# arkworks-rs/circom-compat

Hardware: NVIDIA H100
Metric: groth16_proofs_per_sec_bn254_2p20 (higher is better)
Workload: dtype u32x8 (254-bit Montgomery integers)

## Files before the change

### circom_compat_b200/csrc/msm.cu

```cuda
#include <type_traits>
#include "msm.cuh"
#include "util.cuh"

namespace b2g {

std::atomic<uint64_t> g_launch_count{0};

template <class C, class F>
__global__ void __launch_bounds__(128) msm_table_kernel(const void* __restrict__ bases, uint32_t n, int c, int nwin, void* __restrict__ table) {
    uint32_t i = blockIdx.x * blockDim.x + threadIdx.x;
    if (i >= n) return;
    using Pt = typename C::Pt; using Aff = typename C::Aff; using E = typename F::elem;
    Aff p = aff_load<F>(bases, i);
    if (C::aff_is_inf(p)) {
        Aff z; z.x = F::zero(); z.y = F::zero();
        for (int w = 0; w < nwin; w++) aff_store<F>(table, (size_t)w * n + i, z);
        return;
    }
    Pt pts[MSM_MAX_WIN];
    E pre[MSM_MAX_WIN];
    Pt cur = C::from_affine(p);
    E acc = F::one();
    for (int w = 0; w < nwin; w++) {
        pts[w] = cur;
// ... 81 lines not shown
        if (mine) pending = false;
    }
    if (pending) atomicAdd(&counts[b], 1u);
}

__global__ void __launch_bounds__(1024) msm_scan_kernel(const uint32_t* __restrict__ counts, uint32_t nb, uint32_t* __restrict__ offsets,
                                                        uint32_t* __restrict__ cursor) {
    __shared__ uint32_t warp_sums[32];
    __shared__ uint32_t carry_s;
    const uint32_t tid = threadIdx.x, per = (nb + 1023u) / 1024u;
    const uint32_t lo = tid * per, hi = min(lo + per, nb);
    uint32_t s = 0;
    if ((per & 3u) == 0 && hi == lo + per) {
        const uint4* v4 = reinterpret_cast<const uint4*>(counts + lo);
        #pragma unroll 4
        for (uint32_t j = 0; j < per / 4; j++) { const uint4 q = __ldg(&v4[j]); s += q.x + q.y + q.z + q.w; }
    } else {
        for (uint32_t j = lo; j < hi; j++) s += counts[j];
    }
    uint32_t v = s;
    #pragma unroll
    for (int d = 1; d < 32; d <<= 1) { uint32_t t = __shfl_up_sync(0xffffffffu, v, d); if ((tid & 31) >= (uint32_t)d) v += t; }
    if ((tid & 31) == 31) warp_sums[tid >> 5] = v;
    __syncthreads();
    if (tid < 32) {
        uint32_t w = warp_sums[tid], x = w;
        #pragma unroll
        for (int d = 1; d < 32; d <<= 1) { uint32_t t = __shfl_up_sync(0xffffffffu, x, d); if (tid >= (uint32_t)d) x += t; }
        warp_sums[tid] = x - w;
        if (tid == 31) carry_s = x;
    }
    __syncthreads();
    uint32_t run = warp_sums[tid >> 5] + v - s;
    for (uint32_t j = lo; j < hi; j++) { offsets[j] = run; cursor[j] = 0; run += counts[j]; }
    if (tid == 0) offsets[nb] = carry_s;
}

__global__ void __launch_bounds__(256) msm_scatter_kernel(const fe* __restrict__ canon, uint32_t n, uint32_t row_stride, int c, int nwin, uint32_t nb,
                                   const uint32_t* __restrict__ offsets, uint32_t* __restrict__ cursor, uint32_t* __restrict__ entries) {
    canon += (size_t)blockIdx.y * n;
    offsets += (size_t)blockIdx.y * nb;
    cursor += (size_t)blockIdx.y * nb;
    const uint64_t tid = (uint64_t)blockIdx.x * blockDim.x + threadIdx.x;
    const uint32_t w = (uint32_t)(tid / n), i = (uint32_t)(tid % n);
    int32_t d = 0;
    if (w < (uint32_t)nwin) d = msm_digit_at(canon[i].l, c, (int)w);
    const uint32_t b = d ? (uint32_t)(d < 0 ? -d : d) - 1u : 0xffffffffu;
    const uint32_t lane = threadIdx.x & 31;
    const uint32_t entry = (w * row_stride + i) | (d < 0 ? 0x80000000u : 0u);
    bool pending = d != 0;
    {
        const uint32_t hot = __ballot_sync(0xffffffffu, pending && b == 0u);
        if (hot) {
            const int leader = __ffs(hot) - 1;
            uint32_t base = 0;
            if ((int)lane == leader) base = atomicAdd(&cursor[0], (uint32_t)__popc(hot));
            base = __shfl_sync(0xffffffffu, base, leader);
            if (pending && b == 0u) {
                entries[offsets[0] + base + (uint32_t)__popc(hot & ((1u << lane) - 1u))] = entry;
                pending = false;
            }
        }
    }
    #pragma unroll
    for (int round = 0; round < MSM_LEADER_ROUNDS; round++) {
        const uint32_t pend = __ballot_sync(0xffffffffu, pending);
        if (!pend) break;
        const int leader = __ffs(pend) - 1;
        const uint32_t lb = __shfl_sync(0xffffffffu, b, leader);
        const bool mine = pending && b == lb;
        const uint32_t same = __ballot_sync(0xffffffffu, mine);
        uint32_t base = 0;
        if ((int)lane == leader) base = atomicAdd(&cursor[lb], (uint32_t)__popc(same));
        base = __shfl_sync(0xffffffffu, base, leader);
        if (mine) {
            entries[offsets[b] + base + (uint32_t)__popc(same & ((1u << lane) - 1u))] = entry;
            pending = false;
        }
    }
    if (pending) entries[offsets[b] + atomicAdd(&cursor[b], 1u)] = entry;
}


__device__ __forceinline__ void acc_stage_slab(uint32_t* slab, unsigned long long* slab_bar, const uint32_t* __restrict__ entries,
                                               uint64_t cta_first, uint32_t total, uint32_t slab_words) {
    const uint32_t bar = (uint32_t)__cvta_generic_to_shared(slab_bar);
    if (threadIdx.x == 0) {
        asm volatile("mbarrier.init.shared::cta.b64 [%0], 1;" :: "r"(bar));
        asm volatile("fence.mbarrier_init.release.cluster;" ::: "memory");
    }
    __syncthreads();
    if (threadIdx.x == 0 && cta_first < total) {
        const uint64_t left = total - cta_first;
        const uint32_t bytes = (uint32_t)(((left < slab_words ? left : (uint64_t)slab_words) * 4 + 15) & ~15ull);
        asm volatile("mbarrier.arrive.expect_tx.shared::cta.b64 _, [%0], %1;" :: "r"(bar), "r"(bytes) : "memory");
        asm volatile("cp.async.bulk.shared::cluster.global.mbarrier::complete_tx::bytes [%0], [%1], %2, [%3];"
                     :: "r"((uint32_t)__cvta_generic_to_shared(slab)), "l"(entries + cta_first), "r"(bytes), "r"(bar) : "memory");
    }
    if (cta_first < total) {
        uint32_t done = 0;
        while (!done)
            asm volatile("{\n\t.reg .pred p;\n\tmbarrier.try_wait.parity.shared::cta.b64 p, [%1], 0;\n\tselp.u32 %0, 1, 0, p;\n\t}" : "=r"(done) : "r"(bar) : "memory");
    }
}

constexpr int MSM_SLAB_MAX_BYTES = 48 * 1024;

__device__ __forceinline__ uint32_t acc_first_bucket(const uint32_t* __restrict__ offsets, uint32_t nb, uint32_t start, uint32_t& bucket_end) {
    uint32_t lo = 0, hi = nb;
    while (hi - lo > 1) { uint32_t mid = (lo + hi) >> 1; if (offsets[mid] <= start) lo = mid; else hi = mid; }
    uint32_t b = lo;
    bucket_end = offsets[b + 1];
    while (bucket_end <= start) { b++; bucket_end = offsets[b + 1]; }
    return b;
}

template <class C, class F>
__global__ void __launch_bounds__(128, 4) msm_accumulate_kernel(const void* __restrict__ table, const uint32_t* __restrict__ entries,
                                      const uint32_t* __restrict__ offsets, uint32_t nb, uint32_t chunk,
                                      void* __restrict__ buckets, void* __restrict__ frag_first, void* __restrict__ frag_last, uint32_t slab_words) {
    using Pt = typename C::Pt; using Aff = typename C::Aff;
    const uint32_t total = offsets[nb];
    const uint32_t t = blockIdx.x * blockDim.x + threadIdx.x;
    const uint64_t start64 = (uint64_t)t * chunk;
    extern __shared__ __align__(128) uint32_t slab[];
    __shared__ __align__(8) unsigned long long slab_bar;
    const uint64_t cta_first = (uint64_t)blockIdx.x * blockDim.x * chunk;
    if (slab_words) acc_stage_slab(slab, &slab_bar, entries, cta_first, total, slab_words);
    if (start64 >= total) return;
    const uint32_t start = (uint32_t)start64;
    const uint32_t end = (uint32_t)min((uint64_t)total, start64 + chunk);
    uint32_t bucket_end;
    uint32_t b = acc_first_bucket(offsets, nb, start, bucket_end);
    Pt acc = C::infinity();
    uint32_t seg_start = start;
    for (uint32_t pos = start; pos < end;) {
        const uint32_t e = slab_words ? slab[pos - start + threadIdx.x * chunk] : entries[pos];
        Aff p = aff_load<F>(table, (size_t)(e & 0x7fffffffu));
        if (e >> 31) p.y = F::neg(p.y);
        C::madd(acc, p);
        pos++;
        if (pos == bucket_end || pos == end) {
            const uint32_t bucket_start = offsets[b];
            if (bucket_start >= start && bucket_end <= end) pt_store<F>(buckets, b, acc);
            else if (seg_start == start) pt_store<F>(frag_first, t, acc);
            else pt_store<F>(frag_last, t, acc);
            acc = C::infinity();
            seg_start = pos;
            if (pos == bucket_end && pos < end) {
                do { b++; bucket_end = offsets[b + 1]; } while (bucket_end <= pos);
            }
        }
    }
}

__global__ void __launch_bounds__(128, 3) msm_accumulate_g2_kernel(const void* __restrict__ table, const uint32_t* __restrict__ entries,
                                      const uint32_t* __restrict__ offsets, uint32_t nb, uint32_t chunk,
                                      void* __restrict__ buckets, void* __restrict__ frag_first, void* __restrict__ frag_last) {
    const uint32_t total = offsets[nb];
    const uint32_t t = (blockIdx.x * blockDim.x + threadIdx.x) >> 1;
    const uint32_t half = threadIdx.x & 1u;
    const bool A = half == 0;
    const unsigned mask = 3u << (threadIdx.x & 30u);
    const uint64_t start64 = (uint64_t)t * chunk;
    if (start64 >= total) return;
    const uint32_t start = (uint32_t)start64;
    const uint32_t end = (uint32_t)min((uint64_t)total, start64 + chunk);
    uint32_t bucket_end;
    uint32_t b = acc_first_bucket(offsets, nb, start, bucket_end);
    fe2 s0 = Fq2::zero(), s1 = Fq2::zero();
    bool empty = true;
    uint32_t seg_start = start;
    for (uint32_t pos = start; pos < end;) {
        const uint32_t e = entries[pos];
        fe2 qc;
        elem_load_nc(qc, (const char*)table + (size_t)(e & 0x7fffffffu) * 128 + half * 64);
        qc = Fq2::sel((e >> 31) && !A, Fq2::neg(qc), qc);
        G2Pair::madd(s0, s1, empty, qc, A, mask);
        pos++;
        if (pos == bucket_end || pos == end) {
            const uint32_t bucket_start = offsets[b];
            char* rec;
            if (bucket_start >= start && bucket_end <= end) rec = (char*)buckets + (size_t)b * 256;
            else if (seg_start == start) rec = (char*)frag_first + (size_t)t * 256;
            else rec = (char*)frag_last + (size_t)t * 256;
            elem_store(rec + half * 64, s0);
            elem_store(rec + 128 + half * 64, s1);
            s0 = Fq2::zero(); s1 = Fq2::zero(); empty = true;
            seg_start = pos;
            if (pos == bucket_end && pos < end) {
                do { b++; bucket_end = offsets[b + 1]; } while (bucket_end <= pos);
            }
        }
    }
}


template <class C, class F>
__global__ void __launch_bounds__(128) msm_fold_kernel(const uint32_t* __restrict__ offsets, uint32_t nb, uint32_t chunk, void* __restrict__ buckets,
                                const void* __restrict__ frag_first, const void* __restrict__ frag_last,
                                uint32_t* __restrict__ big_list, uint32_t* __restrict__ big_count) {
    using Pt = typename C::Pt;
    uint32_t b = blockIdx.x * blockDim.x + threadIdx.x;
    if (b >= nb) return;
    uint32_t s = offsets[b], e = offsets[b + 1];
    if (s == e) { pt_store<F>(buckets, b, C::infinity()); return; }
    uint32_t t0 = s / chunk, t1 = (e - 1) / chunk;
    if (t0 == t1) return;
    if (t1 - t0 + 1 > (uint32_t)MSM_BIG_FRAGS) { big_list[atomicAdd(big_count, 1u)] = b; return; }
    Pt acc = (s == t0 * chunk) ? pt_load<F>(frag_first, t0) : pt_load<F>(frag_last, t0);
    for (uint32_t t = t0 + 1; t <= t1; t++) { Pt q = pt_load<F>(frag_first, t); C::add(acc, q); }
    pt_store<F>(buckets, b, acc);
}

template <class F> struct PtWords;
template <> struct PtWords<Fq> { static constexpr int N = 32; };
template <> struct PtWords<Fq2> { static constexpr int N = 64; };

template <class C, class F>
__device__ __forceinline__ typename C::Pt warp_sum_points(typename C::Pt v) {
    using Pt = typename C::Pt;
    static_assert(sizeof(Pt) == PtWords<F>::N * 4, "XYZZ point layout");
    #pragma unroll 1
    for (int d = 16; d > 0; d >>= 1) {
        Pt q;
        uint32_t* qw = reinterpret_cast<uint32_t*>(&q);
        const uint32_t* vw = reinterpret_cast<const uint32_t*>(&v);
        #pragma unroll
        for (int i = 0; i < PtWords<F>::N; i++) qw[i] = __shfl_down_sync(0xffffffffu, vw[i], d);
        if ((int)(threadIdx.x & 31) < d) C::add(v, q);
    }
    return v;
}

template <class C, class F, int NT>
__device__ __forceinline__ typename C::Pt block_sum_points(typename C::Pt v, typename C::Pt* sh) {
    static_assert(NT == 32 || NT == 64, "one or two warps");
    v = warp_sum_points<C, F>(v);
    if (NT == 32) return v;
    if ((threadIdx.x & 31) == 0) sh[threadIdx.x >> 5] = v;
    __syncthreads();
    if (threadIdx.x == 0) { typename C::Pt q = sh[1]; C::add(v, q); }
    __syncthreads();
    return v;
}

template <class F> struct TailThreads;
template <> struct TailThreads<Fq> { static constexpr int N = 64; };
template <> struct TailThreads<Fq2> { static constexpr int N = 32; };
constexpr int MSM_REDUCE_CHUNK_DEFAULT = 8;

template <class C, class F>
__global__ void __launch_bounds__(TailThreads<F>::N) msm_fold_big_kernel(const uint32_t* __restrict__ offsets, uint32_t chunk, void* __restrict__ buckets,
                                    const void* __restrict__ frag_first, const void* __restrict__ frag_last,
                                    const uint32_t* __restrict__ big_list, const uint32_t* __restrict__ big_count) {
    using Pt = typename C::Pt;
    extern __shared__ __align__(32) unsigned char smem_raw[];
    Pt* sh = reinterpret_cast<Pt*>(smem_raw);
    const uint32_t nbig = *big_count;
    for (uint32_t bi = blockIdx.x; bi < nbig; bi += gridDim.x) {
        uint32_t b = big_list[bi];
// ... 28 lines not shown
            C::add(acc, run);
        }
        if (base != 0 && !C::is_inf(run)) {
            Pt m = C::infinity();
            int top = 31 - __clz(base);
            for (int i = top; i >= 0; i--) { m = C::dbl(m); if ((base >> i) & 1u) C::add(m, run); }
            C::add(acc, m);
        }
    }
    Pt r = block_sum_points<C, F, TailThreads<F>::N>(acc, sh);
    if (threadIdx.x == 0) pt_store<F>(partials, blockIdx.x, r);
}

template <class C, class F>
__global__ void __launch_bounds__(TailThreads<F>::N) msm_sum_kernel(const void* __restrict__ pts, uint32_t count, void* __restrict__ out, size_t out_stride) {
    using Pt = typename C::Pt;
    extern __shared__ __align__(32) unsigned char smem_raw[];
    Pt* sh = reinterpret_cast<Pt*>(smem_raw);
    pts = (const char*)pts + (size_t)blockIdx.x * count * sizeof(Pt);
    out = (char*)out + (size_t)blockIdx.x * out_stride;
    Pt acc = C::infinity();
    for (uint32_t i = threadIdx.x; i < count; i += TailThreads<F>::N) { Pt q = pt_load<F>(pts, i); C::add(acc, q); }
    Pt r = block_sum_points<C, F, TailThreads<F>::N>(acc, sh);
    if (threadIdx.x == 0) pt_store<F>(out, 0, r);
}

static uint32_t env_u32(const char* name, uint32_t dflt) {
    const char* v = getenv(name);
    if (!v || !*v) return dflt;
    long x = strtol(v, nullptr, 10);
    return x > 0 ? (uint32_t)x : dflt;
}

void msm_validate_points(const void* pts_dev, uint32_t n, bool g2, cudaStream_t st, const char* what) {
    if (n == 0) return;
    struct Flag { uint32_t* d = nullptr; ~Flag() { if (d) cudaFree(d); } } flag;
    uint32_t bad = 0;
    CUDA_CHECK(cudaMalloc(&flag.d, 4));
    CUDA_CHECK(cudaMemsetAsync(flag.d, 0, 4, st));
    if (g2) msm_validate_kernel<G2, Fq2><<<(n + 255) / 256, 256, 0, st>>>(pts_dev, n, flag.d);
    else msm_validate_kernel<G1, Fq><<<(n + 255) / 256, 256, 0, st>>>(pts_dev, n, flag.d);
    g_launch_count += 1;
    CUDA_CHECK(cudaMemcpyAsync(&bad, flag.d, 4, cudaMemcpyDeviceToHost, st));
    CUDA_CHECK(cudaStreamSynchronize(st));
    if (bad) throw_error(B2G_E_INPUT, std::string(g2 ? "G2" : "G1") + " point " + std::to_string(bad - 1) + " of " + what + " is not on the curve");
}

template <class C, class F>
static void msm_build_table_t(MsmPlan& plan, const void* bases_dev, uint32_t n, cudaStream_t st) {
    const size_t aff = 2 * Bytes<F>::ELEM;
    uint32_t c = env_u32("B2G_MSM_C", (uint32_t)msm_pick_c(n ? n : 1));
    if (c < 8 || c > 22) throw_error(B2G_E_SHAPE, "B2G_MSM_C must be in [8, 22]");
    plan.n = n; plan.c = (int)c; plan.nwin = msm_nwin(plan.c); plan.nbuckets = 1u << (plan.c - 1);
    if (n == 0) { plan.table = nullptr; return; }
    if ((uint64_t)n * plan.nwin >= (1ull << 31)) throw_error(B2G_E_SHAPE, "msm: n * windows exceeds 2^31 table rows");
    msm_validate_points(bases_dev, n, plan.g2, st, "the query slice");
    CUDA_CHECK(cudaMalloc(&plan.table, (size_t)n * plan.nwin * aff));
    msm_table_kernel<C, F><<<(n + 127) / 128, 128, 0, st>>>(bases_dev, n, plan.c, plan.nwin, plan.table);
    g_launch_count += 1;
    CUDA_CHECK(cudaGetLastError());
}

void msm_build_table(MsmPlan& plan, const void* bases_dev, uint32_t n, bool g2, cudaStream_t st) {
    plan.g2 = g2;
    if (g2) msm_build_table_t<G2, Fq2>(plan, bases_dev, n, st);
    else msm_build_table_t<G1, Fq>(plan, bases_dev, n, st);
}

void msm_free_table(MsmPlan& plan) { if (plan.table) cudaFree(plan.table); plan.table = nullptr; }

void msm_scratch_alloc(MsmScratch& s, uint32_t n, int nwin, uint32_t nbuckets_one, bool g2, bool with_sort, uint32_t count) {
    s.g2 = g2; s.cap_n = n; s.cap_nwin = nwin; s.cap_buckets = nbuckets_one; s.cap_count = count;
    s.chunk = env_u32(g2 ? "B2G_MSM_CHUNK_G2" : "B2G_MSM_CHUNK", env_u32("B2G_MSM_CHUNK", 64));
    const size_t pt = (g2 ? 4 * 64 : 4 * 32);
    const size_t nent = (size_t)n * nwin * count;
    const size_t nbuckets = (size_t)nbuckets_one * count;
    const size_t nchunks = (nent + s.chunk - 1) / s.chunk + 1;
    s.reduce_chunk = env_u32("B2G_MSM_REDUCE_CHUNK", MSM_REDUCE_CHUNK_DEFAULT);
    const size_t npart = ((size_t)nbuckets_one / (s.reduce_chunk * 32) + 64) * count;
    if (with_sort) {
        CUDA_CHECK(cudaMalloc(&s.counts, (size_t)nbuckets * 4));
        CUDA_CHECK(cudaMalloc(&s.offsets, ((size_t)nbuckets + 1) * 4));
        CUDA_CHECK(cudaMalloc(&s.cursor, (size_t)nbuckets * 4));
        CUDA_CHECK(cudaMalloc(&s.entries, (nent + 8) * 4));
        CUDA_CHECK(cudaMalloc(&s.scalars_canon, ((size_t)n * count + 1) * sizeof(fe)));
    }
    CUDA_CHECK(cudaMalloc(&s.big_list, (size_t)nbuckets * 4));
    CUDA_CHECK(cudaMalloc(&s.big_count, 4));
    CUDA_CHECK(cudaMalloc(&s.frag_first, nchunks * pt));
    CUDA_CHECK(cudaMalloc(&s.frag_last, nchunks * pt));
    CUDA_CHECK(cudaMalloc(&s.buckets, (size_t)nbuckets * pt));
    CUDA_CHECK(cudaMalloc(&s.partials, (npart + 1) * pt));
    CUDA_CHECK(cudaMalloc(&s.result, pt)); s.result_owned = true;
    int least = 0, greatest = 0;
    CUDA_CHECK(cudaDeviceGetStreamPriorityRange(&least, &greatest));
    CUDA_CHECK(cudaStreamCreateWithPriority(&s.tail, cudaStreamNonBlocking, greatest));
    CUDA_CHECK(cudaEventCreateWithFlags(&s.ev_acc, cudaEventDisableTiming));
    CUDA_CHECK(cudaEventCreateWithFlags(&s.ev_tail, cudaEventDisableTiming));
}

void msm_scratch_free(MsmScratch& s) {
    void* ptrs[] = {s.counts, s.offsets, s.cursor, s.entries, s.big_list, s.big_count, s.frag_first, s.frag_last,
                    s.buckets, s.partials, s.result_owned ? s.result : nullptr, s.scalars_canon};
    for (void* p : ptrs) if (p) cudaFree(p);
    if (s.tail) { cudaStreamDestroy(s.tail); cudaEventDestroy(s.ev_acc); cudaEventDestroy(s.ev_tail); }
    s = MsmScratch();
}

void msm_sort(const MsmPlan& plan, MsmScratch& s, const fe* scalars_dev, uint32_t n, bool scalars_mont, cudaStream_t st, uint32_t count,
              uint32_t scalar_stride) {
    if (n > plan.n) n = plan.n;
    s.sorted_n = n; s.sorted_count = count;
    if (n == 0 || plan.table == nullptr) return;
    if (n > s.cap_n || plan.nwin > s.cap_nwin || plan.nbuckets > s.cap_buckets || count > s.cap_count || !s.entries) throw_error(B2G_E_SHAPE, "msm: sort scratch too small");
    const uint32_t nb = plan.nbuckets * count;
    constexpr unsigned SORT_CTA = 256;
    CUDA_CHECK(cudaMemsetAsync(s.counts, 0, (size_t)nb * 4, st));
    const dim3 pair_grid((unsigned)(((uint64_t)n * plan.nwin + SORT_CTA - 1) / SORT_CTA), count);
    msm_canon_kernel<<<dim3((n + SORT_CTA - 1) / SORT_CTA, count), SORT_CTA, 0, st>>>(scalars_dev, n, scalar_stride ? scalar_stride : n, scalars_mont ? 1 : 0, s.scalars_canon);
    msm_count_kernel<<<pair_grid, SORT_CTA, 0, st>>>(s.scalars_canon, n, plan.c, plan.nwin, plan.nbuckets, s.counts);
    msm_scan_kernel<<<1, 1024, 0, st>>>(s.counts, nb, s.offsets, s.cursor);
    msm_scatter_kernel<<<pair_grid, SORT_CTA, 0, st>>>(s.scalars_canon, n, plan.n, plan.c, plan.nwin, plan.nbuckets, s.offsets, s.cursor, s.entries);
    g_launch_count += 4;
    CUDA_CHECK(cudaGetLastError());
}

template <class C, class F>
static void launch_accumulate(const void* table, const uint32_t* entries, const uint32_t* offsets, uint32_t nb, uint32_t chunk, uint32_t nruns,
                              const MsmScratch& s, cudaStream_t st) {
    constexpr bool g2 = std::is_same<F, Fq2>::value;
    constexpr uint32_t runs_per_cta = g2 ? 64u : 128u;
    const unsigned blocks = (unsigned)(((uint64_t)nruns + runs_per_cta - 1) / runs_per_cta);
    if constexpr (g2) {
        msm_accumulate_g2_kernel<<<blocks, 128, 0, st>>>(table, entries, offsets, nb, chunk, s.buckets, s.frag_first, s.frag_last);
    } else {
        const uint32_t slab_words = (size_t)chunk * runs_per_cta * 4 <= MSM_SLAB_MAX_BYTES ? chunk * runs_per_cta : 0u;
        msm_accumulate_kernel<C, F><<<blocks, 128, (size_t)slab_words * 4, st>>>(table, entries, offsets, nb, chunk, s.buckets, s.frag_first, s.frag_last, slab_words);
    }
}

template <class C, class F>
static void msm_accumulate_t(const MsmPlan& plan, const MsmScratch& sorted, MsmScratch& s, cudaStream_t st) {
    using Pt = typename C::Pt;
    const size_t ptb = sizeof(Pt);
    const uint32_t n = sorted.sorted_n, count = sorted.sorted_count;
    const size_t rstride = s.result_stride ? s.result_stride : ptb;
    if (n == 0 || plan.table == nullptr) { CUDA_CHECK(cudaMemset2DAsync(s.result, rstride, 0, ptb, count, st)); return; }
    if (plan.nbuckets > s.cap_buckets || n > s.cap_n || plan.nwin > s.cap_nwin || count > s.cap_count) throw_error(B2G_E_SHAPE, "msm: accumulate scratch too small");
    const uint32_t nb = plan.nbuckets * count, chunk = s.chunk;
    const uint32_t* offsets = sorted.offsets;
    CUDA_CHECK(cudaMemsetAsync(s.big_count, 0, 4, st));
    const uint64_t nent = (uint64_t)n * plan.nwin * count;
    const uint32_t nthreads = (uint32_t)((nent + chunk - 1) / chunk);
    if (s.prof0) CUDA_CHECK(cudaEventRecord(s.prof0, st));
    launch_accumulate<C, F>(plan.table, sorted.entries, offsets, nb, chunk, nthreads, s, st);
    if (s.prof1) CUDA_CHECK(cudaEventRecord(s.prof1, st));
    cudaStream_t main_st = st;
    CUDA_CHECK(cudaEventRecord(s.ev_acc, st)); CUDA_CHECK(cudaStreamWaitEvent(s.tail, s.ev_acc, 0)); st = s.tail;
    msm_fold_kernel<C, F><<<(nb + 127) / 128, 128, 0, st>>>(offsets, nb, chunk, s.buckets, s.frag_first, s.frag_last, s.big_list, s.big_count);
    constexpr int NT = TailThreads<F>::N;
    const size_t sh = (size_t)NT * ptb;
    msm_fold_big_kernel<C, F><<<128, NT, sh, st>>>(offsets, chunk, s.buckets, s.frag_first, s.frag_last, s.big_list, s.big_count);
    const uint32_t rchunk = s.reduce_chunk, nb1 = plan.nbuckets;
    const uint32_t nred = (nb1 + rchunk - 1) / rchunk;
    const uint32_t npart = (nred + NT - 1) / NT;
    msm_reduce_kernel<C, F><<<dim3(npart, count), NT, sh, st>>>(s.buckets, nb1, rchunk, s.partials);
    msm_sum_kernel<C, F><<<count, NT, sh, st>>>(s.partials, npart, s.result, rstride);
    CUDA_CHECK(cudaEventRecord(s.ev_tail, s.tail)); CUDA_CHECK(cudaStreamWaitEvent(main_st, s.ev_tail, 0));
    g_launch_count += 5;
    CUDA_CHECK(cudaGetLastError());
}

void msm_accumulate(const MsmPlan& plan, const MsmScratch& sorted, MsmScratch& acc, cudaStream_t st) {
    if (plan.g2) msm_accumulate_t<G2, Fq2>(plan, sorted, acc, st);
    else msm_accumulate_t<G1, Fq>(plan, sorted, acc, st);
}

void msm_run(const MsmPlan& plan, MsmScratch& s, const fe* scalars_dev, uint32_t n, bool scalars_mont, cudaStream_t st, uint32_t count,
             uint32_t scalar_stride) {
    msm_sort(plan, s, scalars_dev, n, scalars_mont, st, count, scalar_stride);
    msm_accumulate(plan, s, s, st);
}

constexpr uint32_t POWERS_CHUNK = 16;

__global__ void powers_base_kernel(const fe* __restrict__ rho, uint64_t start, fe* __restrict__ pw) {
    if (threadIdx.x != 0 || blockIdx.x != 0) return;
    const fe r = *rho;
    fe acc = Fr::one(), sq = r;
    for (uint64_t e = start; e; e >>= 1) {
        if (e & 1) acc = Fr::mul(acc, sq);
        sq = Fr::sqr(sq);
    }
    pw[0] = acc;
    fe c = r;
    for (uint32_t k = 1; k < POWERS_CHUNK; k <<= 1) c = Fr::sqr(c);
    pw[1] = c;
}

__global__ void __launch_bounds__(256) powers_scalars_kernel(const fe* __restrict__ rho, const fe* __restrict__ pw, uint32_t n,
                                                             fe* __restrict__ canon) {
    const uint32_t t = blockIdx.x * blockDim.x + threadIdx.x;
    const uint32_t i0 = t * POWERS_CHUNK;
    if (i0 >= n) return;
    fe x = pw[0], sq = pw[1];
    for (uint32_t e = t; e; e >>= 1) {
        if (e & 1) x = Fr::mul(x, sq);
        sq = Fr::sqr(sq);
    }
    const fe r = *rho;
    const uint32_t end = min(n, i0 + POWERS_CHUNK);
    for (uint32_t i = i0; i < end; i++) {
        fe_store(&canon[i], Fr::to_canonical(x));
        x = Fr::mul(x, r);
    }
}

__global__ void __launch_bounds__(256) powers_count_kernel(const fe* __restrict__ canon, uint32_t n, int c, int nwin, uint32_t nb,
                                                           uint32_t* __restrict__ counts) {
    const uint64_t tid = (uint64_t)blockIdx.x * blockDim.x + threadIdx.x;
    const uint32_t w = (uint32_t)(tid / n), i = (uint32_t)(tid % n);
    if (w >= (uint32_t)nwin) return;
    const int32_t d = msm_digit_at(canon[i].l, c, (int)w);
    if (d) atomicAdd(&counts[w * nb + (uint32_t)(d < 0 ? -d : d) - 1u], 1u);
}

__global__ void __launch_bounds__(256) powers_scatter_kernel(const fe* __restrict__ canon, uint32_t n, int c, int nwin, uint32_t nb,
                                                             const uint32_t* __restrict__ offsets, uint32_t* __restrict__ cursor,
                                                             uint32_t* __restrict__ entries) {
    const uint64_t tid = (uint64_t)blockIdx.x * blockDim.x + threadIdx.x;
    const uint32_t w = (uint32_t)(tid / n), i = (uint32_t)(tid % n);
    if (w >= (uint32_t)nwin) return;
    const int32_t d = msm_digit_at(canon[i].l, c, (int)w);
    if (!d) return;
    const uint32_t key = w * nb + (uint32_t)(d < 0 ? -d : d) - 1u;
    entries[offsets[key] + atomicAdd(&cursor[key], 1u)] = i | (d < 0 ? 0x80000000u : 0u);
}

template <class C, class F>
__global__ void powers_horner_kernel(const void* __restrict__ windows, int nwin, int c, void* __restrict__ acc) {
    if (threadIdx.x != 0 || blockIdx.x != 0) return;
    typename C::Pt r = pt_load<F>(windows, nwin - 1);
    for (int w = nwin - 2; w >= 0; w--) {
        for (int k = 0; k < c; k++) r = C::dbl(r);
        C::add(r, pt_load<F>(windows, w));
    }
    typename C::Pt a = pt_load<F>(acc, 0);
    C::add(a, r);
    pt_store<F>(acc, 0, a);
}

void powers_msm_alloc(PowersMsm& m, bool g2, uint32_t cap) {
    m.g2 = g2;
    m.cap = cap ? cap : 1;
    m.c = powers_pick_c(m.cap);
    m.nwin = msm_nwin(m.c);
    m.nbuckets = 1u << (m.c - 1);
    const size_t pt = g2 ? 256 : 128, nb = (size_t)m.nbuckets * m.nwin;
    msm_scratch_alloc(m.s, m.cap, 1, m.nbuckets, g2, false, (uint32_t)m.nwin);
    CUDA_CHECK(cudaMalloc(&m.s.counts, nb * 4));
    CUDA_CHECK(cudaMalloc(&m.s.offsets, (nb + 1) * 4));
    CUDA_CHECK(cudaMalloc(&m.s.cursor, nb * 4));
    CUDA_CHECK(cudaMalloc(&m.s.entries, ((size_t)m.cap * m.nwin + 8) * 4));
    CUDA_CHECK(cudaMalloc(&m.s.scalars_canon, ((size_t)m.cap + POWERS_CHUNK) * sizeof(fe)));
    CUDA_CHECK(cudaFree(m.s.result));
    m.s.result = nullptr;
    CUDA_CHECK(cudaMalloc(&m.s.result, (size_t)m.nwin * pt));
    m.s.result_stride = pt;
    CUDA_CHECK(cudaMalloc(&m.acc, pt));
    CUDA_CHECK(cudaMalloc(&m.pw, 2 * sizeof(fe)));
}

void powers_msm_free(PowersMsm& m) {
    msm_scratch_free(m.s);
    if (m.acc) cudaFree(m.acc);
    if (m.pw) cudaFree(m.pw);
    m = PowersMsm();
}

void powers_msm_reset(PowersMsm& m, cudaStream_t st) { CUDA_CHECK(cudaMemsetAsync(m.acc, 0, m.g2 ? 256 : 128, st)); }

void powers_scalars(const fe* rho, uint64_t start, uint32_t n, fe* pw, fe* canon, cudaStream_t st) {
    if (n == 0) return;
    constexpr unsigned CTA = 256;
    powers_base_kernel<<<1, 1, 0, st>>>(rho, start, pw);
    powers_scalars_kernel<<<(n + POWERS_CHUNK * CTA - 1) / (POWERS_CHUNK * CTA), CTA, 0, st>>>(rho, pw, n, canon);
    g_launch_count += 2;
    CUDA_CHECK(cudaGetLastError());
}

template <class C, class F>
static void powers_msm_slice_t(PowersMsm& m, const void* bases, uint32_t n, uint64_t start, const fe* rho, cudaStream_t st,
                               const fe* scalars) {
    if (n == 0) return;
    if (n > m.cap) throw_error(B2G_E_SHAPE, "powers msm: slice larger than its buffers");
    constexpr unsigned CTA = 256;
    const uint32_t nb = m.nbuckets * (uint32_t)m.nwin;
    if (!scalars) {
        powers_scalars(rho, start, n, m.pw, m.s.scalars_canon, st);
        scalars = m.s.scalars_canon;
    }
    CUDA_CHECK(cudaMemsetAsync(m.s.counts, 0, (size_t)nb * 4, st));
    const unsigned blocks = (unsigned)(((uint64_t)n * m.nwin + CTA - 1) / CTA);
    powers_count_kernel<<<blocks, CTA, 0, st>>>(scalars, n, m.c, m.nwin, m.nbuckets, m.s.counts);
    msm_scan_kernel<<<1, 1024, 0, st>>>(m.s.counts, nb, m.s.offsets, m.s.cursor);
    powers_scatter_kernel<<<blocks, CTA, 0, st>>>(scalars, n, m.c, m.nwin, m.nbuckets, m.s.offsets, m.s.cursor, m.s.entries);
    g_launch_count += 3;
    CUDA_CHECK(cudaGetLastError());
    MsmPlan plan;
    plan.n = n; plan.c = m.c; plan.nwin = 1; plan.nbuckets = m.nbuckets; plan.table = const_cast<void*>(bases); plan.g2 = m.g2;
    m.s.sorted_n = n; m.s.sorted_count = (uint32_t)m.nwin;
    msm_accumulate_t<C, F>(plan, m.s, m.s, st);
    powers_horner_kernel<C, F><<<1, 1, 0, st>>>(m.s.result, m.nwin, m.c, m.acc);
    g_launch_count += 1;
    CUDA_CHECK(cudaGetLastError());
}

void powers_msm_slice(PowersMsm& m, const void* bases, uint32_t n, uint64_t start, const fe* rho, cudaStream_t st, const fe* scalars) {
    if (m.g2) powers_msm_slice_t<G2, Fq2>(m, bases, n, start, rho, st, scalars);
    else powers_msm_slice_t<G1, Fq>(m, bases, n, start, rho, st, scalars);
}

void msm_init_kernels() {
    CUDA_CHECK(cudaFuncSetAttribute(msm_accumulate_kernel<G1, Fq>, cudaFuncAttributeMaxDynamicSharedMemorySize, MSM_SLAB_MAX_BYTES));
}

}
```

### circom_compat_b200/csrc/prover.cu

```cuda
#include <atomic>
#include <chrono>
#include <cstring>
#include <vector>
#include "../../include/b2groth.h"
#include "ec.cuh"
#include "msm.cuh"
#include "fixed.cuh"
#include "ntt.cuh"
#include "setup.cuh"
#include "util.cuh"
#include "verify.cuh"

namespace b2g {

void msm_build_table(MsmPlan& plan, const void* bases_dev, uint32_t n, bool g2, cudaStream_t st);
void msm_free_table(MsmPlan& plan);
void msm_scratch_alloc(MsmScratch& s, uint32_t n, int nwin, uint32_t nbuckets, bool g2, bool with_sort, uint32_t count = 1);
void msm_sort(const MsmPlan& plan, MsmScratch& s, const fe* scalars_dev, uint32_t n, bool scalars_mont, cudaStream_t st, uint32_t count = 1,
              uint32_t scalar_stride = 0);
void msm_accumulate(const MsmPlan& plan, const MsmScratch& sorted, MsmScratch& acc, cudaStream_t st);
void msm_scratch_free(MsmScratch& s);
void msm_run(const MsmPlan& plan, MsmScratch& s, const fe* scalars_dev, uint32_t n, bool scalars_mont, cudaStream_t st, uint32_t count = 1,
             uint32_t scalar_stride = 0);
void msm_init_kernels();
void msm_validate_points(const void* pts_dev, uint32_t n, bool g2, cudaStream_t st, const char* what);

enum { Q_H = 0, Q_L = 1, Q_A = 2, Q_B1 = 3, Q_B2 = 4, NQ = 5 };
static const size_t PARTIAL_OFF[NQ] = {0, 128, 256, 384, 512};
constexpr size_t REC_BYTES = B2G_PARTIAL_BYTES + 256;
constexpr uint32_t MAX_BATCH = 65535;

}

using namespace b2g;

struct b2g_ctx {
    int device = 0, shard_rank = 0, shard_count = 1;
    cudaStream_t st[NQ] = {}, st_glue = nullptr;
    cudaEvent_t ev_w = nullptr, ev_sort = nullptr, ev_pre = nullptr, ev_fork = nullptr, ev_done[NQ] = {}, ev_t[20] = {};
    MsmScratch scratch[NQ];
    bool scratch_ok = false;
    uint32_t cap_batch = 1;
    uint8_t* d_partial = nullptr;
    uint8_t* d_partials_all = nullptr;
    uint8_t* d_proof = nullptr;
    uint8_t* d_pre = nullptr;
    fe *d_w = nullptr, *d_a = nullptr, *d_b = nullptr, *d_c = nullptr, *d_h = nullptr;
    fe* d_wb = nullptr; size_t cap_wb = 0;
    cudaEvent_t ev_sortb = nullptr; bool scratch_bsort = false;
    size_t cap_w = 0, cap_n = 0;
    float last_ms[16] = {};
    bool pre_valid = false; uint32_t pre_r[8] = {}, pre_s[8] = {};
    uint8_t *d_rs = nullptr, *h_rs = nullptr;
    uint8_t *h_proof = nullptr, *pending_out = nullptr;
    uint32_t pending_count = 0;
    bool use_graph = true;
    cudaGraphExec_t gexec[2] = {nullptr, nullptr};
    uint64_t g_key[2][4] = {};
    uint64_t alloc_gen = 1;
    uint64_t g_launches[2] = {0, 0};
    unsigned long long* d_epoch = nullptr;
    uint8_t* d_xchg = nullptr;
    size_t eval_cap = 0, eval_common = 0;
    uint8_t** d_peer_ptrs = nullptr;
    void* peer_mapped[64] = {};
    int peers_imported = 0;
    VerifyBufs* vbufs = nullptr;
};

static std::atomic<uint64_t> g_next_uid{1};

struct b2g_pk {
    uint64_t uid = g_next_uid++;
    int device = 0, shard_rank = 0, shard_count = 1;
    uint32_t n_vars = 0, n_public = 0, domain = 0;
    MsmPlan plan[NQ];
    uint32_t lo[NQ] = {}, cnt[NQ] = {}, scalar_off[NQ] = {};
    uint8_t* d_consts = nullptr;
    void *d_tab_delta1 = nullptr, *d_tab_delta2 = nullptr;
    void *d_tab_aa = nullptr, *d_tab_bb = nullptr;
    uint32_t* d_bidx = nullptr;
    uint32_t b_compact = 0;
};

struct b2g_mat {
    uint64_t uid = g_next_uid++;
    int device = 0;
    uint32_t m = 0, num_inputs = 0, n_vars = 0, n = 0;
    int logn = 0;
    NttDomain dom;
    uint32_t *a_rowptr = nullptr, *a_col = nullptr, *b_rowptr = nullptr, *b_col = nullptr, *c_rowptr = nullptr, *c_col = nullptr;
    fe *a_val = nullptr, *b_val = nullptr, *c_val = nullptr;
    uint32_t reduction = B2G_REDUCTION_CIRCOM;
};

namespace b2g {

thread_local std::string g_last_error;

struct Scalar256 { uint32_t l[8]; };

CtxView ctx_view(b2g_ctx* ctx) { return {ctx->device, ctx->st[0], ctx->pending_out != nullptr, &ctx->vbufs}; }

constexpr size_t PRE_BYTES = 2 * 128 + 256;
__global__ void __launch_bounds__(160) glue_pre_kernel(const void* __restrict__ tab_d1, const void* __restrict__ tab_d2, const void* __restrict__ tab_aa,
                                                       const void* __restrict__ tab_bb, const Scalar256* __restrict__ rs, uint8_t* __restrict__ pre) {
    __shared__ G1::Pt sh1[4][32];
// ... 534 lines not shown
    if (!ctx->use_graph) { enqueue_proof(ctx, pk, mat, kind, true, count); return; }
    const uint64_t key[4] = {pk->uid, mat->uid, ctx->alloc_gen, count};
    if (ctx->gexec[kind] && memcmp(ctx->g_key[kind], key, sizeof key)) { cudaGraphExecDestroy(ctx->gexec[kind]); ctx->gexec[kind] = nullptr; }
    if (!ctx->gexec[kind]) {
        const uint64_t before = g_launch_count.load();
        cudaGraph_t graph = nullptr;
        CUDA_CHECK(cudaStreamBeginCapture(s0, cudaStreamCaptureModeThreadLocal));
        try { enqueue_proof(ctx, pk, mat, kind, false, count); }
        catch (...) { cudaStreamEndCapture(s0, &graph); if (graph) cudaGraphDestroy(graph); cudaGetLastError(); g_launch_count = before; throw; }
        cudaError_t e = cudaStreamEndCapture(s0, &graph);
        if (e == cudaSuccess) e = cudaGraphInstantiate(&ctx->gexec[kind], graph, 0);
        if (graph) cudaGraphDestroy(graph);
        ctx->g_launches[kind] = g_launch_count.load() - before;
        g_launch_count = before;
        if (e != cudaSuccess) {
            cudaGetLastError();
            ctx->gexec[kind] = nullptr; ctx->use_graph = false;
            enqueue_proof(ctx, pk, mat, kind, true, count);
            return;
        }
        memcpy(ctx->g_key[kind], key, sizeof key);
    }
    CUDA_CHECK(cudaEventRecord(ctx->ev_t[10], s0)); CUDA_CHECK(cudaEventRecord(ctx->ev_t[11], s0));
    for (int i = 0; i < 10; i++) CUDA_CHECK(cudaEventRecord(ctx->ev_t[i], s0));
    CUDA_CHECK(cudaGraphLaunch(ctx->gexec[kind], s0));
    CUDA_CHECK(cudaEventRecord(ctx->ev_t[14], s0));
    g_launch_count += ctx->g_launches[kind];
}

static void collect_timings(b2g_ctx* ctx) {
    auto el = [&](int a, int b) { float ms = 0; cudaEventElapsedTime(&ms, ctx->ev_t[a], ctx->ev_t[b]); return ms; };
    ctx->last_ms[0] = el(12, 13);
    ctx->last_ms[1] = el(10, 11);
    ctx->last_ms[2] = el(0, 1);
    for (int q = 1; q < NQ; q++) ctx->last_ms[2 + q] = el(2 * q, 2 * q + 1);
    ctx->last_ms[7] = el(14, 15);
    ctx->last_ms[8] = el(12, 15);
}

}

extern "C" {

const char* b2g_last_error(void) { return g_last_error.c_str(); }
int b2g_version(void) { return 1; }

int b2g_device_count(int* count) {
    return guarded([&] { if (!count) throw_error(B2G_E_SHAPE, "null pointer"); CUDA_CHECK(cudaGetDeviceCount(count)); });
}

int b2g_ctx_create(int device, int shard_rank, int shard_count, b2g_ctx** out) {
    return guarded([&] {
        if (!out) throw_error(B2G_E_SHAPE, "null pointer");
        if (shard_count < 1 || shard_count > 64 || shard_rank < 0 || shard_rank >= shard_count) throw_error(B2G_E_SHAPE, "bad shard rank/count");
        int ndev = 0;
        CUDA_CHECK(cudaGetDeviceCount(&ndev));
        if (device < 0 || device >= ndev) throw_error(B2G_E_DEVICE, "no such CUDA device (this library has no CPU fallback)");
        DevGuard g(device);
        b2g_ctx* ctx = new b2g_ctx();
        ctx->device = device; ctx->shard_rank = shard_rank; ctx->shard_count = shard_count;
        int least = 0, greatest = 0;
        CUDA_CHECK(cudaDeviceGetStreamPriorityRange(&least, &greatest));
        for (int i = 0; i < NQ; i++) { CUDA_CHECK(cudaStreamCreateWithPriority(&ctx->st[i], cudaStreamNonBlocking, least)); CUDA_CHECK(cudaEventCreateWithFlags(&ctx->ev_done[i], cudaEventDisableTiming)); }
        CUDA_CHECK(cudaEventCreateWithFlags(&ctx->ev_w, cudaEventDisableTiming));
        CUDA_CHECK(cudaEventCreateWithFlags(&ctx->ev_sort, cudaEventDisableTiming));
        CUDA_CHECK(cudaEventCreateWithFlags(&ctx->ev_pre, cudaEventDisableTiming));
        CUDA_CHECK(cudaEventCreateWithFlags(&ctx->ev_fork, cudaEventDisableTiming));
        CUDA_CHECK(cudaEventCreateWithFlags(&ctx->ev_sortb, cudaEventDisableTiming));
        CUDA_CHECK(cudaStreamCreateWithPriority(&ctx->st_glue, cudaStreamNonBlocking, least));
        for (auto& e : ctx->ev_t) CUDA_CHECK(cudaEventCreate(&e));
        CUDA_CHECK(cudaMalloc(&ctx->d_partial, REC_BYTES));
        CUDA_CHECK(cudaMemset(ctx->d_partial, 0, REC_BYTES));
        CUDA_CHECK(cudaMalloc(&ctx->d_partials_all, 64 * REC_BYTES));
        CUDA_CHECK(cudaMalloc(&ctx->d_proof, 256));
        CUDA_CHECK(cudaMalloc(&ctx->d_pre, PRE_BYTES));
        CUDA_CHECK(cudaMalloc(&ctx->d_rs, 64));
        CUDA_CHECK(cudaMallocHost(&ctx->h_rs, 64));
        CUDA_CHECK(cudaMallocHost(&ctx->h_proof, 256));
        CUDA_CHECK(cudaMalloc(&ctx->d_epoch, 8));
        CUDA_CHECK(cudaMemset(ctx->d_epoch, 0, 8));
        { const char* g = getenv("B2G_GRAPH"); ctx->use_graph = !(g && *g == '0'); }
        cudaDeviceSetLimit(cudaLimitMaxL2FetchGranularity, 64); cudaGetLastError();
        CUDA_CHECK(cudaMalloc(&ctx->d_peer_ptrs, 64 * sizeof(uint8_t*)));
        msm_init_kernels();
        *out = ctx;
    });
}

int b2g_ctx_destroy(b2g_ctx* ctx) {
    return guarded([&] {
        if (!ctx) return;
        DevGuard g(ctx->device);
        cudaDeviceSynchronize();
        for (int i = 0; i < NQ; i++) { if (ctx->scratch_ok) msm_scratch_free(ctx->scratch[i]); cudaStreamDestroy(ctx->st[i]); cudaEventDestroy(ctx->ev_done[i]); }
        cudaEventDestroy(ctx->ev_w); cudaEventDestroy(ctx->ev_sort); cudaEventDestroy(ctx->ev_pre); cudaEventDestroy(ctx->ev_fork); cudaEventDestroy(ctx->ev_sortb); cudaStreamDestroy(ctx->st_glue);
        if (ctx->d_wb) cudaFree(ctx->d_wb);
        for (auto& g : ctx->gexec) if (g) cudaGraphExecDestroy(g);
        if (ctx->h_rs) cudaFreeHost(ctx->h_rs);
        if (ctx->h_proof) cudaFreeHost(ctx->h_proof);
        if (ctx->d_rs) cudaFree(ctx->d_rs);
        if (ctx->d_epoch) cudaFree(ctx->d_epoch);
        for (auto& e : ctx->ev_t) cudaEventDestroy(e);
        for (int k = 0; k < 64; k++) if (ctx->peer_mapped[k]) cudaIpcCloseMemHandle(ctx->peer_mapped[k]);
        verify_bufs_free(ctx->vbufs);
        for (void* p : {(void*)ctx->d_xchg, (void*)ctx->d_peer_ptrs, (void*)ctx->d_partial, (void*)ctx->d_partials_all, (void*)ctx->d_proof, (void*)ctx->d_pre, (void*)ctx->d_w,
                        (void*)ctx->d_a, (void*)ctx->d_b, (void*)ctx->d_c, (void*)ctx->d_h}) if (p) cudaFree(p);
        delete ctx;
    });
}

int b2g_pk_load(b2g_ctx* ctx, const b2g_pk_desc* d, b2g_pk** out) {
    return guarded([&] {
        if (!ctx || !d || !out) throw_error(B2G_E_SHAPE, "null pointer");
        if (d->n_vars < d->n_public + 1 || d->domain_size == 0) throw_error(B2G_E_SHAPE, "bad proving-key header");
        for (const void* p : {d->alpha_g1, d->beta_g1, d->delta_g1, d->beta_g2, d->delta_g2, d->a_query, d->b_g1_query, d->b_g2_query, d->h_query})
            if (!p) throw_error(B2G_E_SHAPE, "null proving-key section");
        DevGuard g(ctx->device);
        cudaStream_t st = ctx->st[0];
        struct PkGuard {
            b2g_pk* pk = new b2g_pk(); void* tmp = nullptr;
            ~PkGuard() { if (tmp) cudaFree(tmp); if (pk) pk_release(pk); }
        } guard;
        b2g_pk* pk = guard.pk;
        pk->device = ctx->device; pk->shard_rank = ctx->shard_rank; pk->shard_count = ctx->shard_count; pk->n_vars = d->n_vars; pk->n_public = d->n_public; pk->domain = d->domain_size;
        const uint32_t li = d->n_public + 1;
        if (d->n_vars - li && !d->l_query) throw_error(B2G_E_SHAPE, "null proving-key section");
        std::vector<uint8_t> l_padded((size_t)(d->n_vars - 1) * 64, 0);
        if (d->n_vars - li) memcpy(l_padded.data() + (size_t)(li - 1) * 64, d->l_query, (size_t)(d->n_vars - li) * 64);
        const uint32_t total[NQ] = {d->domain_size, d->n_vars - 1, d->n_vars - 1, d->n_vars - 1, d->n_vars - 1};
        const uint32_t base_skip[NQ] = {0, 0, 1, 1, 1};
        const uint32_t soff[NQ] = {0, 1, 1, 1, 1};
        const void* src[NQ] = {d->h_query, l_padded.data(), d->a_query, d->b_g1_query, d->b_g2_query};
        std::vector<uint32_t> bidx;
        std::vector<uint8_t> bpacked[2];
        for (int q = 0; q < NQ; q++) {
            const bool g2 = q == Q_B2;
            const size_t aff = g2 ? 128 : 64;
            const uint64_t R = ctx->shard_count, r = ctx->shard_rank;
            pk->lo[q] = (uint32_t)((uint64_t)total[q] * r / R);
            pk->cnt[q] = (uint32_t)((uint64_t)total[q] * (r + 1) / R) - pk->lo[q];
            pk->scalar_off[q] = soff[q];
            if (total[q] && !src[q]) throw_error(B2G_E_SHAPE, "null proving-key section");
            if (q == Q_B1) {
                const uint8_t* b1 = (const uint8_t*)d->b_g1_query + (size_t)(1 + pk->lo[q]) * 64;
                const uint8_t* b2 = (const uint8_t*)d->b_g2_query + (size_t)(1 + pk->lo[q]) * 128;
                auto nonzero = [](const uint8_t* p, size_t n) { const uint64_t* w = (const uint64_t*)p; uint64_t o = 0; for (size_t i = 0; i < n / 8; i++) o |= w[i]; return o != 0; };
                for (uint32_t i = 0; i < pk->cnt[q]; i++) if (nonzero(b1 + (size_t)i * 64, 64) || nonzero(b2 + (size_t)i * 128, 128)) bidx.push_back(i);
                const char* off = getenv("B2G_NO_B_COMPACT");
                if (!(off && *off == '1') && pk->cnt[q] >= 1024 && (uint64_t)bidx.size() * 5 < (uint64_t)pk->cnt[q] * 4) {
                    pk->b_compact = (uint32_t)bidx.size();
                    bpacked[0].resize(bidx.size() * 64 + 64); bpacked[1].resize(bidx.size() * 128 + 128);
                    for (size_t j = 0; j < bidx.size(); j++) { memcpy(&bpacked[0][j * 64], b1 + (size_t)bidx[j] * 64, 64); memcpy(&bpacked[1][j * 128], b2 + (size_t)bidx[j] * 128, 128); }
                    pk->d_bidx = dev_upload<uint32_t>(bidx.data(), bidx.size() * 4, st);
                } else bidx.clear();
            }
            if (pk->d_bidx && (q == Q_B1 || q == Q_B2)) {
                if (pk->b_compact) guard.tmp = dev_upload<uint8_t>(bpacked[g2 ? 1 : 0].data(), (size_t)pk->b_compact * aff, st);
                msm_build_table(pk->plan[q], guard.tmp, pk->b_compact, g2, st);
                g_launch_count += 1;
                CUDA_CHECK(cudaStreamSynchronize(st));
                if (guard.tmp) { cudaFree(guard.tmp); guard.tmp = nullptr; }
                continue;
            }
            if (pk->cnt[q]) guard.tmp = dev_upload<uint8_t>((const uint8_t*)src[q] + (size_t)(base_skip[q] + pk->lo[q]) * aff, (size_t)pk->cnt[q] * aff, st);
            msm_build_table(pk->plan[q], guard.tmp, pk->cnt[q], g2, st);
            g_launch_count += 1;
            CUDA_CHECK(cudaStreamSynchronize(st));
// ... 578 lines not shown
```

Measured before the change: 42.31.

## Prefetch bucket-accumulate table points through a cp.async shared-memory ring

Replaces the bulk-copy staging of the whole entries slab in the G1 accumulate kernel with a per-thread two-deep cp.async ring. Each thread prefetches the affine points of its next entries into shared memory, and sign bits are kept in a register mask. The G2 accumulate kernel gets the same ring for its half-element loads. The aim is to hide the latency of the random table gathers behind the mixed-addition math, at the cost of extra shared memory per block, per-iteration commit and wait overhead, and reading entries straight from global memory instead of from a staged slab.

```diff
diff --git a/circom_compat_b200/csrc/msm.cu b/circom_compat_b200/csrc/msm.cu
--- a/circom_compat_b200/csrc/msm.cu
+++ b/circom_compat_b200/csrc/msm.cu
@@ -187,29 +187,25 @@
 }
 
 
-__device__ __forceinline__ void acc_stage_slab(uint32_t* slab, unsigned long long* slab_bar, const uint32_t* __restrict__ entries,
-                                               uint64_t cta_first, uint32_t total, uint32_t slab_words) {
-    const uint32_t bar = (uint32_t)__cvta_generic_to_shared(slab_bar);
-    if (threadIdx.x == 0) {
-        asm volatile("mbarrier.init.shared::cta.b64 [%0], 1;" :: "r"(bar));
-        asm volatile("fence.mbarrier_init.release.cluster;" ::: "memory");
-    }
-    __syncthreads();
-    if (threadIdx.x == 0 && cta_first < total) {
-        const uint64_t left = total - cta_first;
-        const uint32_t bytes = (uint32_t)(((left < slab_words ? left : (uint64_t)slab_words) * 4 + 15) & ~15ull);
-        asm volatile("mbarrier.arrive.expect_tx.shared::cta.b64 _, [%0], %1;" :: "r"(bar), "r"(bytes) : "memory");
-        asm volatile("cp.async.bulk.shared::cluster.global.mbarrier::complete_tx::bytes [%0], [%1], %2, [%3];"
-                     :: "r"((uint32_t)__cvta_generic_to_shared(slab)), "l"(entries + cta_first), "r"(bytes), "r"(bar) : "memory");
-    }
-    if (cta_first < total) {
-        uint32_t done = 0;
-        while (!done)
-            asm volatile("{\n\t.reg .pred p;\n\tmbarrier.try_wait.parity.shared::cta.b64 p, [%1], 0;\n\tselp.u32 %0, 1, 0, p;\n\t}" : "=r"(done) : "r"(bar) : "memory");
-    }
-}
-
-constexpr int MSM_SLAB_MAX_BYTES = 48 * 1024;
+constexpr int MSM_ACC_THREADS = 128;
+constexpr int MSM_RING = 2;
+constexpr int MSM_RING_BYTES = MSM_RING * 64 * MSM_ACC_THREADS;
+
+__device__ __forceinline__ uint32_t ring_chunk(uint32_t s, uint32_t k) { return ((s * 4 + k) * MSM_ACC_THREADS + threadIdx.x) * 16; }
+
+__device__ __forceinline__ void ring_fill(uint32_t ring, uint32_t s, const void* src) {
+    #pragma unroll
+    for (uint32_t k = 0; k < 4; k++)
+        asm volatile("cp.async.cg.shared.global [%0], [%1], 16;" :: "r"(ring + ring_chunk(s, k)), "l"((const char*)src + 16 * k) : "memory");
+}
+__device__ __forceinline__ void ring_commit() { asm volatile("cp.async.commit_group;" ::: "memory"); }
+__device__ __forceinline__ void ring_wait() { asm volatile("cp.async.wait_group %0;" :: "n"(MSM_RING - 1) : "memory"); }
+
+__device__ __forceinline__ fe ring_elem(const unsigned char* ring, uint32_t s, uint32_t k) {
+    const uint4 a = *reinterpret_cast<const uint4*>(ring + ring_chunk(s, k)), b = *reinterpret_cast<const uint4*>(ring + ring_chunk(s, k + 1));
+    fe r; r.l[0] = a.x; r.l[1] = a.y; r.l[2] = a.z; r.l[3] = a.w; r.l[4] = b.x; r.l[5] = b.y; r.l[6] = b.z; r.l[7] = b.w;
+    return r;
+}
 
 __device__ __forceinline__ uint32_t acc_first_bucket(const uint32_t* __restrict__ offsets, uint32_t nb, uint32_t start, uint32_t& bucket_end) {
     uint32_t lo = 0, hi = nb;
@@ -221,29 +217,48 @@
 }
 
 template <class C, class F>
-__global__ void __launch_bounds__(128, 4) msm_accumulate_kernel(const void* __restrict__ table, const uint32_t* __restrict__ entries,
+__global__ void __launch_bounds__(MSM_ACC_THREADS, 4) msm_accumulate_kernel(const void* __restrict__ table, const uint32_t* __restrict__ entries,
                                       const uint32_t* __restrict__ offsets, uint32_t nb, uint32_t chunk,
-                                      void* __restrict__ buckets, void* __restrict__ frag_first, void* __restrict__ frag_last, uint32_t slab_words) {
+                                      void* __restrict__ buckets, void* __restrict__ frag_first, void* __restrict__ frag_last) {
     using Pt = typename C::Pt; using Aff = typename C::Aff;
     const uint32_t total = offsets[nb];
     const uint32_t t = blockIdx.x * blockDim.x + threadIdx.x;
     const uint64_t start64 = (uint64_t)t * chunk;
-    extern __shared__ __align__(128) uint32_t slab[];
-    __shared__ __align__(8) unsigned long long slab_bar;
-    const uint64_t cta_first = (uint64_t)blockIdx.x * blockDim.x * chunk;
-    if (slab_words) acc_stage_slab(slab, &slab_bar, entries, cta_first, total, slab_words);
+    extern __shared__ __align__(128) unsigned char ring[];
     if (start64 >= total) return;
     const uint32_t start = (uint32_t)start64;
     const uint32_t end = (uint32_t)min((uint64_t)total, start64 + chunk);
+    const uint32_t ring_s = (uint32_t)__cvta_generic_to_shared(ring);
+    uint32_t signs = 0;
+    const uint32_t* ahead = entries + start + MSM_RING;
+    #pragma unroll
+    for (uint32_t s = 0; s < MSM_RING; s++) {
+        if (start + s < end) {
+            const uint32_t e = __ldg(&entries[start + s]);
+            ring_fill(ring_s, s, (const char*)table + (size_t)(e & 0x7fffffffu) * 64);
+            signs |= (e >> 31) << s;
+        }
+        ring_commit();
+    }
     uint32_t bucket_end;
     uint32_t b = acc_first_bucket(offsets, nb, start, bucket_end);
     Pt acc = C::infinity();
     uint32_t seg_start = start;
     for (uint32_t pos = start; pos < end;) {
-        const uint32_t e = slab_words ? slab[pos - start + threadIdx.x * chunk] : entries[pos];
-        Aff p = aff_load<F>(table, (size_t)(e & 0x7fffffffu));
-        if (e >> 31) p.y = F::neg(p.y);
+        const uint32_t s = (pos - start) % MSM_RING;
+        const bool more = pos + MSM_RING < end;
+        const uint32_t e_next = more ? __ldg(ahead + (pos - start)) : 0u;
+        ring_wait();
+        Aff p;
+        p.x = ring_elem(ring, s, 0); p.y = ring_elem(ring, s, 2);
+        if ((signs >> s) & 1u) p.y = F::neg(p.y);
         C::madd(acc, p);
+        signs &= ~(1u << s);
+        if (more) {
+            ring_fill(ring_s, s, (const char*)table + (size_t)(e_next & 0x7fffffffu) * 64);
+            signs |= (e_next >> 31) << s;
+        }
+        ring_commit();
         pos++;
         if (pos == bucket_end || pos == end) {
             const uint32_t bucket_start = offsets[b];
@@ -259,9 +274,10 @@
     }
 }
 
-__global__ void __launch_bounds__(128, 3) msm_accumulate_g2_kernel(const void* __restrict__ table, const uint32_t* __restrict__ entries,
+__global__ void __launch_bounds__(MSM_ACC_THREADS, 3) msm_accumulate_g2_kernel(const void* __restrict__ table, const uint32_t* __restrict__ entries,
                                       const uint32_t* __restrict__ offsets, uint32_t nb, uint32_t chunk,
                                       void* __restrict__ buckets, void* __restrict__ frag_first, void* __restrict__ frag_last) {
+    extern __shared__ __align__(128) unsigned char ring[];
     const uint32_t total = offsets[nb];
     const uint32_t t = (blockIdx.x * blockDim.x + threadIdx.x) >> 1;
     const uint32_t half = threadIdx.x & 1u;
@@ -271,17 +287,38 @@
     if (start64 >= total) return;
     const uint32_t start = (uint32_t)start64;
     const uint32_t end = (uint32_t)min((uint64_t)total, start64 + chunk);
+    const char* my_table = (const char*)table + half * 64;
+    const uint32_t ring_s = (uint32_t)__cvta_generic_to_shared(ring);
+    uint32_t signs = 0;
+    #pragma unroll
+    for (uint32_t s = 0; s < MSM_RING; s++) {
+        if (start + s < end) {
+            const uint32_t e = __ldg(&entries[start + s]);
+            ring_fill(ring_s, s, my_table + (size_t)(e & 0x7fffffffu) * 128);
+            signs |= (e >> 31) << s;
+        }
+        ring_commit();
+    }
     uint32_t bucket_end;
     uint32_t b = acc_first_bucket(offsets, nb, start, bucket_end);
     fe2 s0 = Fq2::zero(), s1 = Fq2::zero();
     bool empty = true;
     uint32_t seg_start = start;
     for (uint32_t pos = start; pos < end;) {
-        const uint32_t e = entries[pos];
+        const uint32_t s = (pos - start) % MSM_RING;
+        const bool more = pos + MSM_RING < end;
+        const uint32_t e_next = more ? __ldg(&entries[pos + MSM_RING]) : 0u;
+        ring_wait();
         fe2 qc;
-        elem_load_nc(qc, (const char*)table + (size_t)(e & 0x7fffffffu) * 128 + half * 64);
-        qc = Fq2::sel((e >> 31) && !A, Fq2::neg(qc), qc);
+        qc.c0 = ring_elem(ring, s, 0); qc.c1 = ring_elem(ring, s, 2);
+        qc = Fq2::sel(((signs >> s) & 1u) && !A, Fq2::neg(qc), qc);
         G2Pair::madd(s0, s1, empty, qc, A, mask);
+        signs &= ~(1u << s);
+        if (more) {
+            ring_fill(ring_s, s, my_table + (size_t)(e_next & 0x7fffffffu) * 128);
+            signs |= (e_next >> 31) << s;
+        }
+        ring_commit();
         pos++;
         if (pos == bucket_end || pos == end) {
             const uint32_t bucket_start = offsets[b];
@@ -476,7 +513,7 @@
         CUDA_CHECK(cudaMalloc(&s.counts, (size_t)nbuckets * 4));
         CUDA_CHECK(cudaMalloc(&s.offsets, ((size_t)nbuckets + 1) * 4));
         CUDA_CHECK(cudaMalloc(&s.cursor, (size_t)nbuckets * 4));
-        CUDA_CHECK(cudaMalloc(&s.entries, (nent + 8) * 4));
+        CUDA_CHECK(cudaMalloc(&s.entries, (nent + 1) * 4));
         CUDA_CHECK(cudaMalloc(&s.scalars_canon, ((size_t)n * count + 1) * sizeof(fe)));
     }
     CUDA_CHECK(cudaMalloc(&s.big_list, (size_t)nbuckets * 4));
@@ -523,13 +560,12 @@
 static void launch_accumulate(const void* table, const uint32_t* entries, const uint32_t* offsets, uint32_t nb, uint32_t chunk, uint32_t nruns,
                               const MsmScratch& s, cudaStream_t st) {
     constexpr bool g2 = std::is_same<F, Fq2>::value;
-    constexpr uint32_t runs_per_cta = g2 ? 64u : 128u;
+    constexpr uint32_t runs_per_cta = g2 ? MSM_ACC_THREADS / 2 : MSM_ACC_THREADS;
     const unsigned blocks = (unsigned)(((uint64_t)nruns + runs_per_cta - 1) / runs_per_cta);
     if constexpr (g2) {
-        msm_accumulate_g2_kernel<<<blocks, 128, 0, st>>>(table, entries, offsets, nb, chunk, s.buckets, s.frag_first, s.frag_last);
+        msm_accumulate_g2_kernel<<<blocks, MSM_ACC_THREADS, MSM_RING_BYTES, st>>>(table, entries, offsets, nb, chunk, s.buckets, s.frag_first, s.frag_last);
     } else {
-        const uint32_t slab_words = (size_t)chunk * runs_per_cta * 4 <= MSM_SLAB_MAX_BYTES ? chunk * runs_per_cta : 0u;
-        msm_accumulate_kernel<C, F><<<blocks, 128, (size_t)slab_words * 4, st>>>(table, entries, offsets, nb, chunk, s.buckets, s.frag_first, s.frag_last, slab_words);
+        msm_accumulate_kernel<C, F><<<blocks, MSM_ACC_THREADS, MSM_RING_BYTES, st>>>(table, entries, offsets, nb, chunk, s.buckets, s.frag_first, s.frag_last);
     }
 }
 
@@ -655,7 +691,7 @@
     CUDA_CHECK(cudaMalloc(&m.s.counts, nb * 4));
     CUDA_CHECK(cudaMalloc(&m.s.offsets, (nb + 1) * 4));
     CUDA_CHECK(cudaMalloc(&m.s.cursor, nb * 4));
-    CUDA_CHECK(cudaMalloc(&m.s.entries, ((size_t)m.cap * m.nwin + 8) * 4));
+    CUDA_CHECK(cudaMalloc(&m.s.entries, ((size_t)m.cap * m.nwin + 1) * 4));
     CUDA_CHECK(cudaMalloc(&m.s.scalars_canon, ((size_t)m.cap + POWERS_CHUNK) * sizeof(fe)));
     CUDA_CHECK(cudaFree(m.s.result));
     m.s.result = nullptr;
@@ -715,8 +751,4 @@
     else powers_msm_slice_t<G1, Fq>(m, bases, n, start, rho, st, scalars);
 }
 
-void msm_init_kernels() {
-    CUDA_CHECK(cudaFuncSetAttribute(msm_accumulate_kernel<G1, Fq>, cudaFuncAttributeMaxDynamicSharedMemorySize, MSM_SLAB_MAX_BYTES));
-}
-
-}
+}
diff --git a/circom_compat_b200/csrc/prover.cu b/circom_compat_b200/csrc/prover.cu
--- a/circom_compat_b200/csrc/prover.cu
+++ b/circom_compat_b200/csrc/prover.cu
@@ -22,7 +22,6 @@
 void msm_scratch_free(MsmScratch& s);
 void msm_run(const MsmPlan& plan, MsmScratch& s, const fe* scalars_dev, uint32_t n, bool scalars_mont, cudaStream_t st, uint32_t count = 1,
              uint32_t scalar_stride = 0);
-void msm_init_kernels();
 void msm_validate_points(const void* pts_dev, uint32_t n, bool g2, cudaStream_t st, const char* what);
 
 enum { Q_H = 0, Q_L = 1, Q_A = 2, Q_B1 = 3, Q_B2 = 4, NQ = 5 };
@@ -723,7 +722,6 @@
         { const char* g = getenv("B2G_GRAPH"); ctx->use_graph = !(g && *g == '0'); }
         cudaDeviceSetLimit(cudaLimitMaxL2FetchGranularity, 64); cudaGetLastError();
         CUDA_CHECK(cudaMalloc(&ctx->d_peer_ptrs, 64 * sizeof(uint8_t*)));
-        msm_init_kernels();
         *out = ctx;
     });
 }
```

Result: faster. 42.93 (median of 6 runs) (+1.5%).
